# cdglissov/recurrent-flows-msc

Measured on AMD Instinct MI355X. Metric: frames/sec, RFN SM-MNIST 64x64 train step (fwd+bwd+Adam), higher is better.
Workload: dtype f32 (forward convolutions fp32-grade: fused scaled-fp16 split f16x3s / three-piece bf16x6 split; gradient convolutions bf16x3 split MFMA; fp32 accumulate everywhere); 1 GPU; RFN SM-MNIST 64x64 canonical (K=10 L=5 Hd=256 h=200 z=56), global_batch=32, seq_len=20, train step; global_batch=32, seq_len=20, parallelism=dp1

## Files before the change

### include/rfn_hip.h

```cpp
#ifndef RFN_HIP_H
#define RFN_HIP_H

#ifdef __cplusplus
extern "C" {
#endif

typedef void* rfn_stream_t;

int rfn_abi_version(void);
const char* rfn_last_error(void);

int rfn_squeeze2d_f32(const float* x, long x_ns, float* y, long y_ns, int N, int C, int H, int W, int undo,
                      rfn_stream_t stream);

int rfn_channel_stats_f32(const float* x, long x_ns, float* mean, float* var_unbiased, int N, int C, int HW,
                          rfn_stream_t stream);

int rfn_actnorm_invconv_fwd_f32(const float* x, long x_ns, const float* bias, const float* logs, const float* Wm,
                                float* z, long z_ns, int N, int C, int HW, rfn_stream_t stream);
int rfn_actnorm_invconv_bwd_f32(const float* x, long x_ns, const float* bias, const float* logs, const float* Wm,
                                const float* gz, long gz_ns, float* gx, long gx_ns, float* gW, float* gbias,
                                float* glogs, int N, int C, int HW, rfn_stream_t stream);
#define RFN_INVCONV_MAX_STEPS 32
#define RFN_INVCONV_MAX_CHANNELS 96
// ... 180 lines not shown
    const float* w;
    float* packed;
    int Cout, Cin, H, W, transpose, pad_;
} rfn_smallmap_pack_desc;
int rfn_smallmap_pack_batched_bf16x3(const void* descs_host, int n, rfn_stream_t stream);
int rfn_smallmap_dense_bf16x3(const float* a, const float* y, float slope_in, const float* packed, const float* bias,
                              const float* add, int act_out, float slope_out, float* out, float* a_out, int B, int K, int N,
                              int HW, rfn_stream_t stream);

int rfn_smallmap_dense_pair_bf16x3(const float* a0, const float* y0, float slope_in0, const float* packed0,
                                   const float* bias0, const float* add0, int act_out0, float slope_out0, float* out0,
                                   float* a_out0, int K0, int N0, const float* a1, const float* y1, float slope_in1,
                                   const float* packed1, const float* bias1, const float* add1, int act_out1,
                                   float slope_out1, float* out1, float* a_out1, int K1, int N1, int B, int HW,
                                   rfn_stream_t stream);

int rfn_smallmap_conv_bf16x3(const float* in1, long in1_ns, int C1, const float* in2, long in2_ns, int C2,
                             const float* packed, float* out1, long out1_ns, float* out2, long out2_ns, int Cout,
                             int cout_split, int acc1, int N, int H, int W, int ep_mode, const float* p0,
                             const float* p1, int act, rfn_stream_t stream);

long rfn_stepbn_scratch_floats(int S, int B, int C);
int rfn_stepbn_fwd_f32(const float* x, const float* gamma, const float* beta, float* y, float* mean, float* var, float* acc,
                       float* run_mean, float* run_var, const float* coef, const float* coef_u, float decay,
                       long long* num_batches_tracked, int S, int B, int C, int HW, float eps, int act, float slope,
                       rfn_stream_t stream);
int rfn_stepbn_bwd_f32(const float* x, const float* gamma, const float* beta, const float* g, const float* mean,
                       const float* var, float* sums, float* gx, float* ggamma, float* gbeta, int S, int B, int C, int HW,
                       float eps, int act, float slope, int stage, int world, rfn_stream_t stream);
int rfn_stepbn_apply_f32(const float* x, const float* gamma, const float* beta, float* y, const float* mean,
                         const float* var, int S, int B, int C, int HW, float eps, int act, float slope,
                         rfn_stream_t stream);
const char* rfn_stepbn_kernel_label(int S, int B, int C, int HW, int aligned, int bwd);

long rfn_bnflow_scratch_floats(int S, int B, int E, int bwd);
int rfn_bnflow_fwd_f32(const float* x, const float* log_gamma, const float* beta, float* z, float* mean, float* var,
                       float* dl, float* scratch, float* run_mean, float* run_var, const float* coef_mean,
                       const float* coef_var, float decay, int S, int B, int E, float eps, rfn_stream_t stream);
int rfn_bnflow_bwd_f32(const float* x, const float* log_gamma, const float* gz, const float* gdl, const float* mean,
                       const float* var, float* gx, float* g_log_gamma, float* g_beta, float* scratch, int S, int B,
                       int E, rfn_stream_t stream);
int rfn_bnflow_apply_f32(const float* x, const float* log_gamma, const float* beta, const float* run_mean,
                         const float* run_var, float* y, float* dl, int N, int E, int reverse, rfn_stream_t stream);

long rfn_mol_part_floats(int N, int HW);
int rfn_mol_nll_fwd(const float* x, const float* l, float* nll_pix, float* lse, float* nll, float* part, int N, int C, int M,
                    int HW, rfn_stream_t stream);
int rfn_mol_nll_bwd(const float* x, const float* l, const float* lse, const float* up, int up_per_pixel, float* dl, int N,
                    int C, int M, int HW, rfn_stream_t stream);
int rfn_mol_sample(const float* l, const float* u_mix, const float* u_x, float* out, int N, int C, int M, int HW,
                   rfn_stream_t stream);
int rfn_mol_sample_keyed(const float* l, float* out, int rows, int B, int C, int M, int HW, long seed, int step,
                         long first_seq, long first_draw, rfn_stream_t stream);
int rfn_mol_keyed_uniforms(float* u_mix, float* u_x, int rows, int B, int C, int M, int HW, long seed, int step,
                           long first_seq, long first_draw, rfn_stream_t stream);

const char* rfn_latent_step_kernel_label(int B, int ZHW);
const char* rfn_convlstm_gates_kernel_label(int N, int Hc, int HW);
int rfn_convlstm_gates_fwd_f32(const float* cc, const float* c_prev, long c_ns, const float* Wci, const float* Wcf,
                               const float* Wco, float* h_out, long h_ns, float* c_out, long co_ns, float* gates,
                               int N, int Hc, int HW, rfn_stream_t stream);
int rfn_convlstm_gates_bwd_f32(const float* gates, const float* c_prev, long c_ns, const float* c_out, long co_ns,
                               const float* gh, long gh_ns, const float* gc_next, long gcn_ns, const float* Wci,
                               const float* Wcf, const float* Wco, float* gcc, float* gc_prev, long gcp_ns, int N,
                               int Hc, int HW, rfn_stream_t stream);

// ... 72 lines not shown
```

### recurrent-flows-msc_amd/Utils/modules.py

```python
import os
from types import SimpleNamespace

import torch
import torch.nn as nn
import torch.nn.functional as F

from rfn_hip import ops as K


class ActFun(nn.Module):

    def __init__(self, non_lin, in_place=False):
        super().__init__()
        if non_lin == "relu":
            self.net = nn.ReLU(inplace=in_place)
        elif non_lin == "leakyrelu":
            self.net = nn.LeakyReLU(negative_slope=0.20, inplace=in_place)
        else:
            assert False, "Please specify a activation type from the set {relu,leakyrelu}"
        self.non_lin = non_lin

    def forward(self, x):
        return self.net(x)

# ... 38 lines not shown
            m = bn.momentum if bn.momentum is not None else 0.1
            coef = m * (1.0 - m) ** torch.arange(steps - 1, -1, -1, device=x.device, dtype=x.dtype)
            decay = (1.0 - m) ** steps
            bn.running_mean.mul_(decay).add_((coef.view(steps, 1) * tmp_m.view(steps, C)).sum(0))
            bn.running_var.mul_(decay).add_((coef.view(steps, 1) * tmp_v.view(steps, C)).sum(0))
            bn.num_batches_tracked += steps
    return y


def _act_code(m):
    if isinstance(m, ActFun):
        m = m.net
    if isinstance(m, nn.LeakyReLU):
        return 2, float(m.negative_slope)
    if isinstance(m, nn.ReLU):
        return 1, 0.0
    if isinstance(m, nn.Tanh):
        return 3, 0.0
    return None


_EMA_COEF = {}


def _ema_coef(steps, m, n, device):
    key = (steps, float(m), int(n), str(device))
    if key not in _EMA_COEF:
        c = m * (1.0 - m) ** torch.arange(steps - 1, -1, -1, dtype=torch.float64)
        _EMA_COEF[key] = (c.to(device=device, dtype=torch.float32),
                          (c * (n / max(n - 1, 1))).to(device=device, dtype=torch.float32))
    return _EMA_COEF[key]


def per_step_batchnorm_act(bn, x, steps, act_code, slope):
    running = None
    if bn.track_running_stats:
        n = (x.shape[0] // steps) * x.shape[2] * x.shape[3]
        m = bn.momentum if bn.momentum is not None else 0.1
        coef, coef_u = _ema_coef(steps, m, n, x.device)
        running = (bn.running_mean, bn.running_var, coef, coef_u, (1.0 - m) ** steps, bn.num_batches_tracked)
    y, _, _ = K.StepBatchNormActFn.apply(x, bn.weight if bn.affine else None, bn.bias if bn.affine else None, steps,
                                         float(bn.eps), act_code, slope, running)
    return y


def queue_conv_packs(seqs, x):
    packs = {}
    if x.is_cuda and x.dtype == torch.float32 and K.CONV_PRECISION != "f32" and K.bwd_b3():
        with K.PackBatch() as pb:
            for seq in seqs:
                for m in seq:
                    if _own_conv(m, x) and not K.fewcin_ok(x, None, m.weight, 0):
                        packs[m] = (pb.conv(m.weight, prec="bf16x6"),
                                    pb.conv(m.weight, flip=True) if torch.is_grad_enabled() else None)
    return packs


def run_time_batched(seq, x, steps, packs=None):
    mods = list(seq)
    if packs is None:
        packs = queue_conv_packs([seq], x)
    i = 0
    while i < len(mods):
        m = mods[i]
        if isinstance(m, NormLayer) and isinstance(m.norm, nn.BatchNorm2d):
            bn = m.norm
            fused = x.is_cuda and bn.training and x.dtype == torch.float32 and os.environ.get("RFN_STEPBN") != "0"
            if fused:
                act = _act_code(mods[i + 1]) if i + 1 < len(mods) else None
                x = per_step_batchnorm_act(bn, x, steps, act[0] if act else 0, act[1] if act else 0.0)
                i += 2 if act else 1
                continue
            x = per_step_batchnorm(bn, x, steps)
        elif _own_conv(m, x):
            x = K.conv_ep(x.contiguous(), None, m.weight, None, None, 0, 0,
                          prec="f32" if K.CONV_PRECISION == "f32" else "bf16x6", packs=packs.get(m))
        else:
            x = m(x)
        i += 1
    return x


def _own_conv(m, x):
    return (isinstance(m, nn.Conv2d) and x.is_cuda and x.dtype == torch.float32
            and tuple(m.kernel_size) == (3, 3) and tuple(m.stride) == (1, 1) and tuple(m.padding) == (1, 1)
            and tuple(m.dilation) == (1, 1) and m.groups == 1 and m.bias is None
            and os.environ.get("RFN_VGG_CONV", "own") != "miopen")


class Squeeze2dDecoder(nn.Module):

    def __init__(self, undo_squeeze=False):
        super().__init__()
        self.undo_squeeze = undo_squeeze

    def forward(self, x):
        return K.Squeeze2dFn.apply(x.contiguous(), self.undo_squeeze)


class _NearestUp2xFn(torch.autograd.Function):

    @staticmethod
    def forward(ctx, x):
        return torch.nn.functional.interpolate(x, scale_factor=2, mode="nearest")

    @staticmethod
    def backward(ctx, g):
        return torch.nn.functional.avg_pool2d(g, 2) * 4.0


class NearestUp2x(nn.Upsample):

    def __init__(self):
        super().__init__(scale_factor=2, mode="nearest")

    def forward(self, x):
        return _NearestUp2xFn.apply(x)


class tanh0_5(nn.Module):
    def forward(self, x):
        return 0.5 * torch.tanh(x)


def _conv_block(cin, cout, norm_type, act, stride=1):
    return [nn.Conv2d(cin, cout, kernel_size=3, stride=stride, padding=1, bias=False),
            NormLayer(cout, norm_type=norm_type), act]


class VGG_downscaler(nn.Module):

    def __init__(self, structures, L, in_channels, norm_type="batchnorm", non_lin="relu", scale=2, skip_con=False,
                 tanh=False):
        super().__init__()
        assert len(structures) == L, "Please specify number of blocks = L"
        self.l_nets = nn.ModuleList([])
        self.L, self.skip_con, self.scale = L, skip_con, scale
        for l, structure in enumerate(structures):
            layers = []
            for count, item in enumerate(structure, 1):
                last = count == len(structure)
                if l == L - 1 and last:
                    act = nn.Tanh()
                elif last and tanh:
                    act = tanh0_5()
                else:
                    act = ActFun(non_lin, in_place=True)
                if item == "pool":
                    layers.append(nn.MaxPool2d(kernel_size=2, stride=2))
                elif item == "conv":
# ... 71 lines not shown
                    in_channels = dc
                elif item == "squeeze":
                    dc = in_channels // 4
                    layer_up = [Squeeze2dDecoder(undo_squeeze=True), NormLayer(dc, norm_type=norm_type), act]
                    in_channels = dc
                else:
                    layers += [nn.Conv2d(in_channels + skip_channels, item, kernel_size=3, stride=1, padding=1,
                                         bias=False), NormLayer(item, norm_type=norm_type), act]
                    in_channels = item
            if l > 0:
                self.upscales_nets.append(nn.Sequential(*layer_up))
            self.net = nn.Sequential(*layers)
            self.l_nets.append(self.net)

    def forward(self, x, skip_list=None):
        outputs = []
        rev = list(reversed(skip_list)) if self.skips else None
        for i in range(self.L):
            if i > 0:
                x = self.upscales_nets[i - 1](x)
            if self.skips:
                x = self.l_nets[i](torch.cat((x, rev[i]), dim=1))
            else:
                x = self.l_nets[i](x)
            outputs.append(x)
        outputs.reverse()
        return outputs

    def forward_steps(self, x, steps, skip_list=None):
        outputs = []
        rev = list(reversed(skip_list)) if self.skips else None
        packs = queue_conv_packs(list(self.upscales_nets) + list(self.l_nets), x)
        for i in range(self.L):
            if i > 0:
                x = run_time_batched(self.upscales_nets[i - 1], x, steps, packs)
            if self.skips:
                x = torch.cat((x, rev[i]), dim=1)
            x = run_time_batched(self.l_nets[i], x, steps, packs)
            outputs.append(x)
        outputs.reverse()
        return outputs


class _StepStash:

    def __init__(self):
        self.xs, self.gs = [], []


class _WeightPort(torch.autograd.Function):

    @staticmethod
    def forward(ctx, w, b, stash):
        ctx.set_materialize_grads(False)
        ctx.stash, ctx.has_bias = stash, b is not None
        ctx.save_for_backward(w)
        return w.view_as(w), (b.view_as(b) if b is not None else None)

    @staticmethod
    def backward(ctx, _gw, _gb):
        (w,) = ctx.saved_tensors
        st = ctx.stash
        if not st.gs:
            return None, None, None
        X = st.xs[0] if len(st.xs) == 1 else torch.cat(st.xs, 0)
        G = st.gs[0] if len(st.gs) == 1 else torch.cat(st.gs, 0)
        st.xs, st.gs = [], []
        _, gw, gb = torch.ops.aten.convolution_backward(G, X, w, [w.shape[0]] if ctx.has_bias else None, [1, 1], [1, 1],
                                                        [1, 1], False, [0, 0], 1, [False, True, ctx.has_bias])
        return gw, (gb if ctx.has_bias else None), None
# ... 328 lines not shown
```

### recurrent-flows-msc_amd/csrc/shell.hip

```cpp
#include "common.h"
#include "../../include/rfn_hip.h"
#include <stdarg.h>

static thread_local char g_err[512] = "";
void rfn_set_error(const char* fmt, ...) {
    va_list ap;
    va_start(ap, fmt);
    vsnprintf(g_err, sizeof(g_err), fmt, ap);
    va_end(ap);
}
extern "C" const char* rfn_last_error(void) { return g_err; }
extern "C" int rfn_abi_version(void) { return 2; }

#include <map>
#include <mutex>
#include <vector>
float* rfn_workspace(hipStream_t s, size_t floats) {
    static std::mutex mu;
    static std::map<int, std::pair<float*, size_t>> tab;
    std::lock_guard<std::mutex> lock(mu);
    int dev = 0;
    (void)hipGetDevice(&dev);
    auto& e = tab[dev];
    if (e.second >= floats) return e.first;
// ... 1580 lines not shown
    if (threadIdx.x == 0) {
        float* dst = acc + ((long)blockIdx.y * gridDim.x + blockIdx.x) * 2;
        dst[0] = ta;
        dst[1] = tv;
    }
}
struct StepBnFused {
    const float* acc;
    float* mean_out;
    float* var_out;
    float* run_mean;
    float* run_var;
    const float* coef;
    const float* coef_u;
    float decay;
    long long* nbt;
    int S, ny;
};
__device__ __forceinline__ void stepbn_moments(const float* __restrict__ x, const float* __restrict__ acc, int sc, int s,
                                               int c, int B, int C, int HW, int ny, int SC, float& m, float& v) {
    if (!acc) return;
    const float K = x[((long)s * B * C + c) * HW];
    const float n = (float)B * HW;
    float s1 = 0.f, s2 = 0.f;
    for (int y = 0; y < ny; ++y) {
        s1 += acc[((long)y * SC + sc) * 2];
        s2 += acc[((long)y * SC + sc) * 2 + 1];
    }
    const float m1 = s1 / n;
    m = K + m1;
    const float vv = s2 / n - m1 * m1;
    v = vv > 0.f ? vv : 0.f;
}
template <int VEC>
__global__ void stepbn_apply_kernel(const float* __restrict__ x, const float* __restrict__ gamma,
                                    const float* __restrict__ beta, float* __restrict__ y, unsigned total, int B, int C,
                                    int HW, float eps, int act, float slope, StepBnFused f) {
    const int SC = f.S * C;
    const unsigned nblk = gridDim.x - 1, bid = blockIdx.x - 1;
    if (blockIdx.x == 0) {
        if (!f.acc) return;
        for (int sc = threadIdx.x; sc < SC; sc += blockDim.x) {
            float m, v;
            stepbn_moments(x, f.acc, sc, sc / C, sc % C, B, C, HW, f.ny, SC, m, v);
            f.mean_out[sc] = m;
            f.var_out[sc] = v;
        }
        if (f.run_mean) {
            for (int c = threadIdx.x; c < C; c += blockDim.x) {
                float em = 0.f, ev = 0.f;
#pragma unroll 4
                for (int s = 0; s < f.S; ++s) {
                    float m, v;
                    stepbn_moments(x, f.acc, s * C + c, s, c, B, C, HW, f.ny, SC, m, v);
                    em = fmaf(f.coef[s], m, em);
                    ev = fmaf(f.coef_u[s], v, ev);
                }
                f.run_mean[c] = fmaf(f.decay, f.run_mean[c], em);
                f.run_var[c] = fmaf(f.decay, f.run_var[c], ev);
            }
        }
        if (f.nbt && threadIdx.x == 0) *f.nbt += f.S;
        return;
    }
    const unsigned nvec = total / VEC;
    for (unsigned iv = bid * blockDim.x + threadIdx.x; iv < nvec; iv += nblk * blockDim.x) {
        const unsigned idx = iv * VEC;
        const unsigned r = idx / (unsigned)HW;
        const int c = (int)(r % (unsigned)C);
        const int s = (int)(r / (unsigned)C / (unsigned)B);
        float m = f.acc ? 0.f : f.mean_out[s * C + c], vr = f.acc ? 0.f : f.var_out[s * C + c];
        stepbn_moments(x, f.acc, s * C + c, s, c, B, C, HW, f.ny, SC, m, vr);
        const float rstd = rsqrtf(vr + eps);
        const float ga = gamma ? gamma[c] : 1.f, be = gamma ? beta[c] : 0.f;
        float v[VEC];
        if (VEC == 4) {
            const float4 t = *reinterpret_cast<const float4*>(x + idx);
            v[0] = t.x; v[1 % VEC] = t.y; v[2 % VEC] = t.z; v[3 % VEC] = t.w;
        } else {
            v[0] = x[idx];
        }
#pragma unroll
        for (int j = 0; j < VEC; ++j) v[j] = stepbn_act((v[j] - m) * rstd * ga + be, act, slope);
        if (VEC == 4)
            *reinterpret_cast<float4*>(y + idx) = float4{v[0], v[1 % VEC], v[2 % VEC], v[3 % VEC]};
        else
            y[idx] = v[0];
    }
}
__global__ __launch_bounds__(256) void stepbn_bwd_reduce_kernel(const float* __restrict__ x,
                                                                const float* __restrict__ gamma,
                                                                const float* __restrict__ beta,
                                                                const float* __restrict__ g,
                                                                const float* __restrict__ mean,
                                                                const float* __restrict__ var, float* __restrict__ sg,
// ... 8 lines not shown
    if ((HW & 3) == 0 && ((((uintptr_t)x) | ((uintptr_t)g)) & 15) == 0) {
        const int HW4 = HW >> 2, nb = (B - (int)blockIdx.y + (int)gridDim.y - 1) / (int)gridDim.y;
        for (int idx = threadIdx.x; idx < nb * HW4; idx += 256) {
            const int bi = idx / HW4, p = idx - bi * HW4;
            const long e0 = off + (blockIdx.y + (long)bi * gridDim.y) * fs;
            const float4 xq = reinterpret_cast<const float4*>(x + e0)[p], gq = reinterpret_cast<const float4*>(g + e0)[p];
            const float xv[4] = {xq.x, xq.y, xq.z, xq.w}, gv[4] = {gq.x, gq.y, gq.z, gq.w};
#pragma unroll
            for (int i = 0; i < 4; ++i) {
                const float xh = (xv[i] - m) * rstd;
                const float gp = gv[i] * stepbn_dact(xh * ga + be, act, slope);
                a += gp;
                ax = fmaf(gp, xh, ax);
            }
        }
    } else {
        for (int b = blockIdx.y; b < B; b += gridDim.y) {
            const long e0 = off + b * fs;
            for (int p = threadIdx.x; p < HW; p += 256) {
                const float xh = (x[e0 + p] - m) * rstd;
                const float gp = g[e0 + p] * stepbn_dact(xh * ga + be, act, slope);
                a += gp;
                ax = fmaf(gp, xh, ax);
            }
        }
    }
    const float ta = block_sum_256(a, sm);
    const float tx = block_sum_256(ax, sm);
    if (threadIdx.x == 0) {
        sg[(long)blockIdx.y * gridDim.x + blockIdx.x] = ta;
        sgx[(long)blockIdx.y * gridDim.x + blockIdx.x] = tx;
    }
}
template <int VEC>
__global__ void stepbn_bwd_apply_kernel(const float* __restrict__ x, const float* __restrict__ beta,
                                        const float* __restrict__ g, const float* __restrict__ mean,
                                        const float* __restrict__ var, const float* __restrict__ gamma,
                                        const float* __restrict__ sg, const float* __restrict__ sgx,
                                        float* __restrict__ gx, unsigned total, int B, int C, int HW, float eps, int act,
                                        float slope, float* __restrict__ ggamma, float* __restrict__ gbeta, int S, int ny,
                                        int world) {
    const int SC = S * C;
    const unsigned nblk = ggamma ? gridDim.x - 1 : gridDim.x, bid = ggamma ? blockIdx.x - 1 : blockIdx.x;
    if (ggamma && blockIdx.x == 0) {
        for (int c = threadIdx.x; c < C; c += blockDim.x) {
            float a = 0.f, b = 0.f;
            for (int i = 0; i < ny * S; ++i) {
                a += sgx[(long)i * C + c];
                b += sg[(long)i * C + c];
            }
            ggamma[c] = a / (float)world;
            gbeta[c] = b / (float)world;
        }
        return;
    }
    const float inv_n = 1.f / ((float)(B * HW) * (float)world);
    const unsigned nvec = total / VEC;
    for (unsigned iv = bid * blockDim.x + threadIdx.x; iv < nvec; iv += nblk * blockDim.x) {
        const unsigned idx = iv * VEC;
        const unsigned r = idx / (unsigned)HW;
        const int c = (int)(r % (unsigned)C);
        const int s = (int)(r / (unsigned)C / (unsigned)B);
        const int sc = s * C + c;
        const float rstd = rsqrtf(var[sc] + eps), m = mean[sc];
        const float w = gamma ? gamma[c] : 1.f, be = gamma ? beta[c] : 0.f;
        float k1 = 0.f, k2 = 0.f;
        for (int yy = 0; yy < ny; ++yy) {
            k1 += sg[(long)yy * SC + sc];
            k2 += sgx[(long)yy * SC + sc];
        }
        k1 *= inv_n;
        k2 *= inv_n;
        float xv[VEC], gv[VEC];
        if (VEC == 4) {
            const float4 t = *reinterpret_cast<const float4*>(x + idx);
            const float4 u = *reinterpret_cast<const float4*>(g + idx);
            xv[0] = t.x; xv[1 % VEC] = t.y; xv[2 % VEC] = t.z; xv[3 % VEC] = t.w;
            gv[0] = u.x; gv[1 % VEC] = u.y; gv[2 % VEC] = u.z; gv[3 % VEC] = u.w;
        } else {
            xv[0] = x[idx];
            gv[0] = g[idx];
        }
#pragma unroll
        for (int j = 0; j < VEC; ++j) {
            const float xh = (xv[j] - m) * rstd;
            const float gp = gv[j] * stepbn_dact(xh * w + be, act, slope);
// ... 84 lines not shown
        hipLaunchKernelGGL(stepbn_apply_kernel<1>, dim3(grid + 1), dim3(256), 0, (hipStream_t)stream, x, gamma, beta, y,
                           (unsigned)total, B, C, HW, eps, act, slope, f);
    RFN_LAUNCH_CHECK();
    return 0;
}
extern "C" int rfn_stepbn_bwd_f32(const float* x, const float* gamma, const float* beta, const float* g, const float* mean,
                                  const float* var, float* sums, float* gx, float* ggamma, float* gbeta, int S, int B,
                                  int C, int HW, float eps, int act, float slope, int stage, int world,
                                  rfn_stream_t stream) {
    RFN_CHECK_ARG(x && g && mean && var && sums && gx && S > 0 && B > 0 && C > 0 && HW > 0, -1);
    RFN_CHECK_ARG(stage >= 0 && stage <= 2 && world >= 1, -4);
    RFN_CHECK_ARG(((gamma && beta) || (!gamma && !beta)) && ((ggamma && gbeta) || (!ggamma && !gbeta)), -2);
    const long total = (long)S * B * C * HW;
    RFN_CHECK_ARG(total < (1L << 31), -3);
    hipStream_t st = (hipStream_t)stream;
    const StepBnRoute r = choose_stepbn(S, B, C, HW, stepbn_aligned(x, g, x, g, gx));
    const int ny = r.ny, grid = r.grid;
    float* sg = sums;
    float* sgx = sums + (long)ny * S * C;
    if (stage != 2)
        hipLaunchKernelGGL(stepbn_bwd_reduce_kernel, dim3(S * C, ny), dim3(256), 0, st, x, gamma, beta, g, mean, var, sg, sgx,
                           B, C, HW, eps, act, slope);
    if (stage == 1) {
        RFN_LAUNCH_CHECK();
        return 0;
    }
    const int extra = ggamma ? 1 : 0;
    if (r.v4)
        hipLaunchKernelGGL(stepbn_bwd_apply_kernel<4>, dim3(grid + extra), dim3(256), 0, st, x, beta, g, mean, var, gamma,
                           sg, sgx, gx, (unsigned)total, B, C, HW, eps, act, slope, ggamma, gbeta, S, ny, world);
    else
        hipLaunchKernelGGL(stepbn_bwd_apply_kernel<1>, dim3(grid + extra), dim3(256), 0, st, x, beta, g, mean, var, gamma,
                           sg, sgx, gx, (unsigned)total, B, C, HW, eps, act, slope, ggamma, gbeta, S, ny, world);
    RFN_LAUNCH_CHECK();
    return 0;
}

struct InvConvWeightsParams {
    const float* p[RFN_INVCONV_MAX_STEPS];
    const float* lower[RFN_INVCONV_MAX_STEPS];
    const float* upper[RFN_INVCONV_MAX_STEPS];
    const float* log_s[RFN_INVCONV_MAX_STEPS];
    const float* sign_s[RFN_INVCONV_MAX_STEPS];
    float* W;
    float* logdet;
    const float* gW;
    const float* gc;
    float* g_lower;
    float* g_upper;
    float* g_log_s;
    int C;
    float hw;
};
__device__ __forceinline__ void invconv_load_LU(const InvConvWeightsParams& q, int k, float* Lm, float* Um) {
    const int C = q.C, CP = C + 1;
    for (int i = threadIdx.x; i < C * C; i += blockDim.x) {
        const int r = i / C, c = i - r * C;
        Lm[r * CP + c] = r > c ? q.lower[k][i] : (r == c ? 1.f : 0.f);
        Um[r * CP + c] = r < c ? q.upper[k][i] : (r == c ? q.sign_s[k][r] * expf(q.log_s[k][r]) : 0.f);
    }
}
__device__ __forceinline__ void invconv_load(const float* __restrict__ src, float* dst, int C) {
    for (int i = threadIdx.x; i < C * C; i += blockDim.x) dst[(i / C) * (C + 1) + i % C] = src[i];
}
template <bool TA, bool TB, typename Store>
__device__ __forceinline__ void invconv_mm(const float* __restrict__ A, const float* __restrict__ B, int C, Store store) {
// ... 318 lines not shown
```

### recurrent-flows-msc_amd/rfn_hip/ops.py

```python
import collections
import ctypes
import functools
import itertools

import torch

from . import lib as L

import os

CONV_PRECISION = os.environ.get("RFN_CONV_PRECISION", "mixed")


def bwd_b3():
    return CONV_PRECISION in ("bf16x3", "mixed")


MIXED_FWD = os.environ.get("RFN_MIXED_FWD", "bf16x6")


def fwd_prec(H, W):
    if CONV_PRECISION == "mixed":
        return "bf16x3" if H * W <= 4 else MIXED_FWD
    return CONV_PRECISION
# ... 1480 lines not shown
            n = B * HW * world
            cfu_g = cf * (n / max(n - 1, 1))
            rm.mul_(decay).add_((cf.view(-1, 1) * mean).sum(0))
            rv.mul_(decay).add_((cfu_g.view(-1, 1) * var).sum(0))
            if nbt is not None:
                nbt.add_(S)
        ctx.save_for_backward(x, mean, var, gm, bt)
        ctx.cfg = (S, B, C, HW, eps, act, slope, gamma is not None, nscr)
        ctx.world = world
        ctx.mark_non_differentiable(mean, var)
        return y, mean, var

    @staticmethod
    def backward(ctx, g, _gm, _gv):
        x, mean, var, gm, bt = ctx.saved_tensors
        S, B, C, HW, eps, act, slope, affine, nscr = ctx.cfg
        if g is None:
            return (None,) * 8
        g = g.contiguous()
        sums = torch.empty((nscr,), device=x.device, dtype=torch.float32)
        gx = torch.empty_like(x)
        ggamma = torch.empty((C,), device=x.device, dtype=torch.float32) if affine else None
        gbeta = torch.empty((C,), device=x.device, dtype=torch.float32) if affine else None
        args = (L.dev(x), L.dev(gm), L.dev(bt), L.dev(g), L.dev(mean), L.dev(var), L.dev(sums), L.dev(gx), L.dev(ggamma),
                L.dev(gbeta), S, B, C, HW, eps, act, slope)
        if ctx.world > 1:
            from . import dist as rdist
            L.call("rfn_stepbn_bwd_f32", *args, 1, ctx.world)
            rdist.all_reduce_sum_(sums)
            L.call("rfn_stepbn_bwd_f32", *args, 2, ctx.world)
        else:
            L.call("rfn_stepbn_bwd_f32", *args, 0, 1)
        return gx, ggamma, gbeta, None, None, None, None, None


def bnflow_coef(steps, momentum):
    m = float(momentum)
    coef = (1.0 - m) * torch.tensor([m ** (steps - 1 - s) for s in range(steps)], dtype=torch.float64)
    return coef, m ** steps


class BatchNormFlowFn(torch.autograd.Function):

    @staticmethod
    def forward(ctx, x, log_gamma, beta, steps, eps, running=None):
        x = x.contiguous()
        S, B = int(steps), int(x.shape[0]) // int(steps)
        E = x[0].numel()
        if S * B != x.shape[0] or log_gamma.numel() != E or beta.numel() != E:
            raise RuntimeError("BatchNormFlowFn: x %s is not %d steps of rows of %d elements" % (tuple(x.shape), S, log_gamma.numel()))
        lg, bt = _f(log_gamma), _f(beta)
        z = torch.empty_like(x)
        mean = torch.empty((S, E), device=x.device, dtype=torch.float32)
        var = torch.empty((S, E), device=x.device, dtype=torch.float32)
        dl = torch.empty((S,), device=x.device, dtype=torch.float32)
        scr = torch.empty((int(L.load().rfn_bnflow_scratch_floats(S, B, E, 0)),), device=x.device, dtype=torch.float32)
        rm = rv = cf = None
        decay = 1.0
        if running is not None:
            rm, rv, cf, decay = running
            if not (rm.is_contiguous() and rv.is_contiguous()) or rm.numel() != E or rv.numel() != E or cf.numel() != S:
                raise RuntimeError("BatchNormFlowFn: running statistics must be dense [%d] tensors, coef [%d]" % (E, S))
        L.call("rfn_bnflow_fwd_f32", L.dev(x), L.dev(lg), L.dev(bt), L.dev(z), L.dev(mean), L.dev(var), L.dev(dl),
               L.dev(scr), L.dev(rm), L.dev(rv), L.dev(cf), L.dev(cf), decay, S, B, E,
               eps, meta=_shell("bnflow_fwd", x, 2))
        ctx.save_for_backward(x, lg, mean, var)
# ... 460 lines not shown
```

Before: 11790 frames/s.

## Fuse per-step BatchNorm+activation with 2x2 maxpool and upsample with skip concat

Adds fused kernels that apply per-step batchnorm, the activation and a 2x2 max-pool in one pass, recomputing the pooling argmax in backward instead of materialising the full-resolution activation. A second fused kernel performs nearest 2x upsampling and channel concatenation with the skip tensor in a single write, with a matching backward that sums the 2x2 gradient blocks. The goal is to cut intermediate full-size tensors and extra kernel launches in the encoder and decoder paths. In exchange, backward recomputes the normalisation and winner selection, and both paths are gated on layer patterns and environment variables.

```diff
diff --git a/include/rfn_hip.h b/include/rfn_hip.h
--- a/include/rfn_hip.h
+++ b/include/rfn_hip.h
@@ -236,6 +236,19 @@
                          const float* var, int S, int B, int C, int HW, float eps, int act, float slope,
                          rfn_stream_t stream);
 const char* rfn_stepbn_kernel_label(int S, int B, int C, int HW, int aligned, int bwd);
+int rfn_stepbn_pool_fwd_f32(const float* x, const float* gamma, const float* beta, float* p, float* mean, float* var,
+                            float* acc, float* run_mean, float* run_var, const float* coef, const float* coef_u,
+                            float decay, long long* num_batches_tracked, int S, int B, int C, int H, int W, float eps,
+                            int act, float slope, rfn_stream_t stream);
+int rfn_stepbn_pool_bwd_f32(const float* x, const float* gamma, const float* beta, const float* gp, const float* mean,
+                            const float* var, float* sums, float* gx, float* ggamma, float* gbeta, int S, int B, int C,
+                            int H, int W, float eps, int act, float slope, int stage, int world, rfn_stream_t stream);
+const char* rfn_stepbn_pool_kernel_label(int S, int B, int C, int H, int W, int aligned, int bwd);
+
+int rfn_up2x_cat_f32(const float* x, long x_ns, const float* skip, long skip_ns, float* out, int N, int Cx, int Cs, int h,
+                     int w, rfn_stream_t stream);
+int rfn_up2x_cat_bwd_f32(const float* g, long g_ns, float* gx, int N, int Cx, int h, int w, rfn_stream_t stream);
+const char* rfn_up2x_cat_kernel_label(int N, int Cx, int Cs, int h, int w, int aligned, int bwd);
 
 long rfn_bnflow_scratch_floats(int S, int B, int E, int bwd);
 int rfn_bnflow_fwd_f32(const float* x, const float* log_gamma, const float* beta, float* z, float* mean, float* var,
diff --git a/recurrent-flows-msc_amd/Utils/modules.py b/recurrent-flows-msc_amd/Utils/modules.py
--- a/recurrent-flows-msc_amd/Utils/modules.py
+++ b/recurrent-flows-msc_amd/Utils/modules.py
@@ -94,15 +94,31 @@
     return _EMA_COEF[key]
 
 
-def per_step_batchnorm_act(bn, x, steps, act_code, slope):
+def _pool2x2(m):
+    pair = lambda v: tuple(v) if isinstance(v, (tuple, list)) else (v, v)
+    return (type(m) is nn.MaxPool2d and pair(m.kernel_size) == (2, 2) and pair(m.stride) == (2, 2)
+            and pair(m.padding) == (0, 0) and pair(m.dilation) == (1, 1) and not m.ceil_mode and not m.return_indices)
+
+
+def _pool_fusable(mods, i, x):
+    if os.environ.get("RFN_STEPBN_POOL") == "0" or i + 2 >= len(mods) or _act_code(mods[i + 1]) is None:
+        return False
+    if not _pool2x2(mods[i + 2]) or x.shape[2] % 2 or x.shape[3] % 2:
+        return False
+    from rfn_hip import dist as rdist
+    return not rdist.sync_batchnorm_on()
+
+
+def per_step_batchnorm_act(bn, x, steps, act_code, slope, pool=False):
     running = None
     if bn.track_running_stats:
         n = (x.shape[0] // steps) * x.shape[2] * x.shape[3]
         m = bn.momentum if bn.momentum is not None else 0.1
         coef, coef_u = _ema_coef(steps, m, n, x.device)
         running = (bn.running_mean, bn.running_var, coef, coef_u, (1.0 - m) ** steps, bn.num_batches_tracked)
-    y, _, _ = K.StepBatchNormActFn.apply(x, bn.weight if bn.affine else None, bn.bias if bn.affine else None, steps,
-                                         float(bn.eps), act_code, slope, running)
+    fn = K.StepBatchNormActPoolFn if pool else K.StepBatchNormActFn
+    y, _, _ = fn.apply(x, bn.weight if bn.affine else None, bn.bias if bn.affine else None, steps, float(bn.eps),
+                       act_code, slope, running)
     return y
 
 
@@ -130,8 +146,9 @@
             fused = x.is_cuda and bn.training and x.dtype == torch.float32 and os.environ.get("RFN_STEPBN") != "0"
             if fused:
                 act = _act_code(mods[i + 1]) if i + 1 < len(mods) else None
-                x = per_step_batchnorm_act(bn, x, steps, act[0] if act else 0, act[1] if act else 0.0)
-                i += 2 if act else 1
+                pool = _pool_fusable(mods, i, x)
+                x = per_step_batchnorm_act(bn, x, steps, act[0] if act else 0, act[1] if act else 0.0, pool)
+                i += 3 if pool else 2 if act else 1
                 continue
             x = per_step_batchnorm(bn, x, steps)
         elif _own_conv(m, x):
@@ -178,6 +195,13 @@
 
     def forward(self, x):
         return _NearestUp2xFn.apply(x)
+
+
+def _up2x_only(seq, x, skip):
+    return (len(seq) == 1 and type(seq[0]) is NearestUp2x and x.is_cuda and skip.is_cuda and x.dtype == torch.float32
+            and skip.dtype == torch.float32 and x.dim() == 4 and skip.dim() == 4 and skip.shape[1] > 0
+            and tuple(skip.shape[2:]) == (2 * x.shape[2], 2 * x.shape[3]) and skip.shape[0] == x.shape[0]
+            and os.environ.get("RFN_UP2X_CAT") != "0")
 
 
 class tanh0_5(nn.Module):
@@ -315,10 +339,13 @@
         rev = list(reversed(skip_list)) if self.skips else None
         packs = queue_conv_packs(list(self.upscales_nets) + list(self.l_nets), x)
         for i in range(self.L):
-            if i > 0:
-                x = run_time_batched(self.upscales_nets[i - 1], x, steps, packs)
-            if self.skips:
-                x = torch.cat((x, rev[i]), dim=1)
+            if i > 0 and self.skips and _up2x_only(self.upscales_nets[i - 1], x, rev[i]):
+                x = K.Up2xCatFn.apply(x, rev[i])
+            else:
+                if i > 0:
+                    x = run_time_batched(self.upscales_nets[i - 1], x, steps, packs)
+                if self.skips:
+                    x = torch.cat((x, rev[i]), dim=1)
             x = run_time_batched(self.l_nets[i], x, steps, packs)
             outputs.append(x)
         outputs.reverse()
diff --git a/recurrent-flows-msc_amd/csrc/shell.hip b/recurrent-flows-msc_amd/csrc/shell.hip
--- a/recurrent-flows-msc_amd/csrc/shell.hip
+++ b/recurrent-flows-msc_amd/csrc/shell.hip
@@ -1636,6 +1636,31 @@
     const float vv = s2 / n - m1 * m1;
     v = vv > 0.f ? vv : 0.f;
 }
+__device__ __forceinline__ void stepbn_finalise(const float* __restrict__ x, int B, int C, int HW, const StepBnFused& f) {
+    const int SC = f.S * C;
+    if (!f.acc) return;
+    for (int sc = threadIdx.x; sc < SC; sc += blockDim.x) {
+        float m, v;
+        stepbn_moments(x, f.acc, sc, sc / C, sc % C, B, C, HW, f.ny, SC, m, v);
+        f.mean_out[sc] = m;
+        f.var_out[sc] = v;
+    }
+    if (f.run_mean) {
+        for (int c = threadIdx.x; c < C; c += blockDim.x) {
+            float em = 0.f, ev = 0.f;
+#pragma unroll 4
+            for (int s = 0; s < f.S; ++s) {
+                float m, v;
+                stepbn_moments(x, f.acc, s * C + c, s, c, B, C, HW, f.ny, SC, m, v);
+                em = fmaf(f.coef[s], m, em);
+                ev = fmaf(f.coef_u[s], v, ev);
+            }
+            f.run_mean[c] = fmaf(f.decay, f.run_mean[c], em);
+            f.run_var[c] = fmaf(f.decay, f.run_var[c], ev);
+        }
+    }
+    if (f.nbt && threadIdx.x == 0) *f.nbt += f.S;
+}
 template <int VEC>
 __global__ void stepbn_apply_kernel(const float* __restrict__ x, const float* __restrict__ gamma,
                                     const float* __restrict__ beta, float* __restrict__ y, unsigned total, int B, int C,
@@ -1643,28 +1668,7 @@
     const int SC = f.S * C;
     const unsigned nblk = gridDim.x - 1, bid = blockIdx.x - 1;
     if (blockIdx.x == 0) {
-        if (!f.acc) return;
-        for (int sc = threadIdx.x; sc < SC; sc += blockDim.x) {
-            float m, v;
-            stepbn_moments(x, f.acc, sc, sc / C, sc % C, B, C, HW, f.ny, SC, m, v);
-            f.mean_out[sc] = m;
-            f.var_out[sc] = v;
-        }
-        if (f.run_mean) {
-            for (int c = threadIdx.x; c < C; c += blockDim.x) {
-                float em = 0.f, ev = 0.f;
-#pragma unroll 4
-                for (int s = 0; s < f.S; ++s) {
-                    float m, v;
-                    stepbn_moments(x, f.acc, s * C + c, s, c, B, C, HW, f.ny, SC, m, v);
-                    em = fmaf(f.coef[s], m, em);
-                    ev = fmaf(f.coef_u[s], v, ev);
-                }
-                f.run_mean[c] = fmaf(f.decay, f.run_mean[c], em);
-                f.run_var[c] = fmaf(f.decay, f.run_var[c], ev);
-            }
-        }
-        if (f.nbt && threadIdx.x == 0) *f.nbt += f.S;
+        stepbn_finalise(x, B, C, HW, f);
         return;
     }
     const unsigned nvec = total / VEC;
@@ -1739,6 +1743,19 @@
         sgx[(long)blockIdx.y * gridDim.x + blockIdx.x] = tx;
     }
 }
+__device__ __forceinline__ void stepbn_param_grads(const float* __restrict__ sg, const float* __restrict__ sgx,
+                                                   float* __restrict__ ggamma, float* __restrict__ gbeta, int C, int S,
+                                                   int ny, int world) {
+    for (int c = threadIdx.x; c < C; c += blockDim.x) {
+        float a = 0.f, b = 0.f;
+        for (int i = 0; i < ny * S; ++i) {
+            a += sgx[(long)i * C + c];
+            b += sg[(long)i * C + c];
+        }
+        ggamma[c] = a / (float)world;
+        gbeta[c] = b / (float)world;
+    }
+}
 template <int VEC>
 __global__ void stepbn_bwd_apply_kernel(const float* __restrict__ x, const float* __restrict__ beta,
                                         const float* __restrict__ g, const float* __restrict__ mean,
@@ -1750,15 +1767,7 @@
     const int SC = S * C;
     const unsigned nblk = ggamma ? gridDim.x - 1 : gridDim.x, bid = ggamma ? blockIdx.x - 1 : blockIdx.x;
     if (ggamma && blockIdx.x == 0) {
-        for (int c = threadIdx.x; c < C; c += blockDim.x) {
-            float a = 0.f, b = 0.f;
-            for (int i = 0; i < ny * S; ++i) {
-                a += sgx[(long)i * C + c];
-                b += sg[(long)i * C + c];
-            }
-            ggamma[c] = a / (float)world;
-            gbeta[c] = b / (float)world;
-        }
+        stepbn_param_grads(sg, sgx, ggamma, gbeta, C, S, ny, world);
         return;
     }
     const float inv_n = 1.f / ((float)(B * HW) * (float)world);
@@ -1909,6 +1918,375 @@
     else
         hipLaunchKernelGGL(stepbn_bwd_apply_kernel<1>, dim3(grid + extra), dim3(256), 0, st, x, beta, g, mean, var, gamma,
                            sg, sgx, gx, (unsigned)total, B, C, HW, eps, act, slope, ggamma, gbeta, S, ny, world);
+    RFN_LAUNCH_CHECK();
+    return 0;
+}
+
+__device__ __forceinline__ int stepbn_pool_winner(const float xv[4], float m, float rstd, float ga, float be, int act,
+                                                  float slope, float& best, float& xh_w, float& u_w) {
+    int k = 0;
+#pragma unroll
+    for (int j = 0; j < 4; ++j) {
+        const float xh = (xv[j] - m) * rstd;
+        const float u = xh * ga + be;
+        const float a = stepbn_act(u, act, slope);
+        if (j == 0 || a > best || isnan(a)) {
+            best = a;
+            xh_w = xh;
+            u_w = u;
+            k = j;
+        }
+    }
+    return k;
+}
+template <int VEC>
+__device__ __forceinline__ void stepbn_pool_load(const float* __restrict__ x, unsigned in0, int W, float xv[2][4]) {
+    if (VEC == 4) {
+        const float4 r0 = *reinterpret_cast<const float4*>(x + in0);
+        const float4 r1 = *reinterpret_cast<const float4*>(x + in0 + W);
+        xv[0][0] = r0.x; xv[0][1] = r0.y; xv[0][2] = r1.x; xv[0][3] = r1.y;
+        xv[1][0] = r0.z; xv[1][1] = r0.w; xv[1][2] = r1.z; xv[1][3] = r1.w;
+    } else {
+        xv[0][0] = x[in0]; xv[0][1] = x[in0 + 1]; xv[0][2] = x[in0 + W]; xv[0][3] = x[in0 + W + 1];
+    }
+}
+template <int VEC>
+__global__ void stepbn_pool_apply_kernel(const float* __restrict__ x, const float* __restrict__ gamma,
+                                         const float* __restrict__ beta, float* __restrict__ p, unsigned nunits, int B,
+                                         int C, int H, int W, float eps, int act, float slope, StepBnFused f) {
+    constexpr int NW = VEC == 4 ? 2 : 1;
+    const int SC = f.S * C, HW = H * W;
+    const unsigned nblk = gridDim.x - 1, bid = blockIdx.x - 1;
+    if (blockIdx.x == 0) {
+        stepbn_finalise(x, B, C, HW, f);
+        return;
+    }
+    const unsigned upr = (unsigned)W / (2 * NW), Ho = (unsigned)H / 2;
+    for (unsigned u = bid * blockDim.x + threadIdx.x; u < nunits; u += nblk * blockDim.x) {
+        const unsigned q = u / upr;
+        const unsigned r = q / Ho;
+        const int c = (int)(r % (unsigned)C);
+        const int s = (int)(r / (unsigned)C / (unsigned)B);
+        float m = f.acc ? 0.f : f.mean_out[s * C + c], vr = f.acc ? 0.f : f.var_out[s * C + c];
+        stepbn_moments(x, f.acc, s * C + c, s, c, B, C, HW, f.ny, SC, m, vr);
+        const float rstd = rsqrtf(vr + eps);
+        const float ga = gamma ? gamma[c] : 1.f, be = gamma ? beta[c] : 0.f;
+        float xv[2][4], o[NW];
+        stepbn_pool_load<VEC>(x, q * 2u * (unsigned)W + 2u * NW * (u - q * upr), W, xv);
+#pragma unroll
+        for (int w = 0; w < NW; ++w) {
+            float xh, uu;
+            stepbn_pool_winner(xv[w], m, rstd, ga, be, act, slope, o[w], xh, uu);
+        }
+        if (VEC == 4)
+            *reinterpret_cast<float2*>(p + 2u * u) = float2{o[0], o[NW - 1]};
+        else
+            p[u] = o[0];
+    }
+}
+__device__ __forceinline__ double block_sum_256_f64(double v, double* sm ) {
+#pragma unroll
+    for (int o = 32; o > 0; o >>= 1) v += __shfl_xor(v, o, 64);
+    const int lane = threadIdx.x & 63, wave = threadIdx.x >> 6;
+    __syncthreads();
+    if (lane == 0) sm[wave] = v;
+    __syncthreads();
+    return (sm[0] + sm[1]) + (sm[2] + sm[3]);
+}
+template <int VEC>
+__global__ __launch_bounds__(256) void stepbn_pool_bwd_reduce_kernel(
+    const float* __restrict__ x, const float* __restrict__ gamma, const float* __restrict__ beta,
+    const float* __restrict__ gp, const float* __restrict__ mean, const float* __restrict__ var, float* __restrict__ sg,
+    float* __restrict__ sgx, int B, int C, int H, int W, float eps, int act, float slope) {
+    constexpr int NW = VEC == 4 ? 2 : 1;
+    __shared__ double sm[4];
+    const int s = blockIdx.x / C, c = blockIdx.x - s * C;
+    const int HW = H * W, upr = W / (2 * NW), upf = (H / 2) * upr;
+    const unsigned pl0 = (unsigned)(s * B) * C + c;
+    const float m = mean[blockIdx.x], rstd = rsqrtf(var[blockIdx.x] + eps);
+    const float ga = gamma ? gamma[c] : 1.f, be = gamma ? beta[c] : 0.f;
+    double a = 0., ax = 0.;
+    const int nb = (B - (int)blockIdx.y + (int)gridDim.y - 1) / (int)gridDim.y;
+    for (int idx = threadIdx.x; idx < nb * upf; idx += 256) {
+        const int bi = idx / upf, t = idx - bi * upf;
+        const unsigned pl = pl0 + (blockIdx.y + (unsigned)bi * gridDim.y) * (unsigned)C;
+        const int i = t / upr, j = t - i * upr;
+        float xv[2][4], gv[NW];
+        stepbn_pool_load<VEC>(x, pl * (unsigned)HW + 2u * i * W + 2u * NW * j, W, xv);
+        const unsigned o0 = pl * (unsigned)(HW / 4) + (unsigned)t * NW;
+        if (VEC == 4) {
+            const float2 g2 = *reinterpret_cast<const float2*>(gp + o0);
+            gv[0] = g2.x; gv[NW - 1] = g2.y;
+        } else {
+            gv[0] = gp[o0];
+        }
+#pragma unroll
+        for (int w = 0; w < NW; ++w) {
+            float best, xh, u;
+            stepbn_pool_winner(xv[w], m, rstd, ga, be, act, slope, best, xh, u);
+            const float g1 = gv[w] * stepbn_dact(u, act, slope);
+            a += (double)g1;
+            ax = fma((double)g1, (double)xh, ax);
+        }
+    }
+    const float ta = (float)block_sum_256_f64(a, sm);
+    const float tx = (float)block_sum_256_f64(ax, sm);
+    if (threadIdx.x == 0) {
+        sg[(long)blockIdx.y * gridDim.x + blockIdx.x] = ta;
+        sgx[(long)blockIdx.y * gridDim.x + blockIdx.x] = tx;
+    }
+}
+template <int VEC>
+__global__ void stepbn_pool_bwd_apply_kernel(const float* __restrict__ x, const float* __restrict__ beta,
+                                             const float* __restrict__ gp, const float* __restrict__ mean,
+                                             const float* __restrict__ var, const float* __restrict__ gamma,
+                                             const float* __restrict__ sg, const float* __restrict__ sgx,
+                                             float* __restrict__ gx, unsigned nunits, int B, int C, int H, int W,
+                                             float eps, int act, float slope, float* __restrict__ ggamma,
+                                             float* __restrict__ gbeta, int S, int ny, int world) {
+    constexpr int NW = VEC == 4 ? 2 : 1;
+    const int SC = S * C, HW = H * W;
+    const unsigned nblk = ggamma ? gridDim.x - 1 : gridDim.x, bid = ggamma ? blockIdx.x - 1 : blockIdx.x;
+    if (ggamma && blockIdx.x == 0) {
+        stepbn_param_grads(sg, sgx, ggamma, gbeta, C, S, ny, world);
+        return;
+    }
+    const float inv_n = 1.f / ((float)(B * HW) * (float)world);
+    const unsigned upr = (unsigned)W / (2 * NW), Ho = (unsigned)H / 2;
+    for (unsigned u = bid * blockDim.x + threadIdx.x; u < nunits; u += nblk * blockDim.x) {
+        const unsigned q = u / upr;
+        const unsigned r = q / Ho;
+        const int c = (int)(r % (unsigned)C);
+        const int s = (int)(r / (unsigned)C / (unsigned)B);
+        const int sc = s * C + c;
+        const float rstd = rsqrtf(var[sc] + eps), m = mean[sc];
+        const float w = gamma ? gamma[c] : 1.f, be = gamma ? beta[c] : 0.f;
+        float k1 = 0.f, k2 = 0.f;
+        for (int yy = 0; yy < ny; ++yy) {
+            k1 += sg[(long)yy * SC + sc];
+            k2 += sgx[(long)yy * SC + sc];
+        }
+        k1 *= inv_n;
+        k2 *= inv_n;
+        const unsigned in0 = q * 2u * (unsigned)W + 2u * NW * (u - q * upr);
+        float xv[2][4], gv[NW];
+        stepbn_pool_load<VEC>(x, in0, W, xv);
+        if (VEC == 4) {
+            const float2 g2 = *reinterpret_cast<const float2*>(gp + 2u * u);
+            gv[0] = g2.x; gv[NW - 1] = g2.y;
+        } else {
+            gv[0] = gp[u];
+        }
+#pragma unroll
+        for (int ww = 0; ww < NW; ++ww) {
+            float best, xhw, uw;
+            const int k = stepbn_pool_winner(xv[ww], m, rstd, w, be, act, slope, best, xhw, uw);
+            const float g1 = gv[ww] * stepbn_dact(uw, act, slope);
+#pragma unroll
+            for (int j = 0; j < 4; ++j) {
+                const float xh = (xv[ww][j] - m) * rstd;
+                const float gpos = j == k ? g1 : 0.f;
+                xv[ww][j] = w * rstd * (gpos - k1 - xh * k2);
+            }
+        }
+        if (VEC == 4) {
+            *reinterpret_cast<float4*>(gx + in0) = float4{xv[0][0], xv[0][1], xv[NW - 1][0], xv[NW - 1][1]};
+            *reinterpret_cast<float4*>(gx + in0 + W) = float4{xv[0][2], xv[0][3], xv[NW - 1][2], xv[NW - 1][3]};
+        } else {
+            gx[in0] = xv[0][0]; gx[in0 + 1] = xv[0][1]; gx[in0 + W] = xv[0][2]; gx[in0 + W + 1] = xv[0][3];
+        }
+    }
+}
+constexpr int STEPBN_POOL_GRID_CAP = 8192;
+struct StepBnPoolRoute {
+    int ny;
+    bool stats_vec;
+    bool v4;
+    long nunits;
+    int grid;
+    int sweeps;
+};
+static StepBnPoolRoute choose_stepbn_pool(int S, int B, int C, int H, int W, int aligned, int bwd) {
+    StepBnPoolRoute r;
+    const long total = (long)S * B * C * H * W;
+    r.ny = stepbn_split(S, B, C);
+    r.stats_vec = (aligned & 1) && (bwd ? W % 4 == 0 : true);
+    r.v4 = W % 4 == 0 && (aligned & 2);
+    r.nunits = r.v4 ? total / 8 : total / 4;
+    const long nb = (r.nunits + 255) / 256;
+    r.grid = (int)(nb < STEPBN_POOL_GRID_CAP ? nb : STEPBN_POOL_GRID_CAP);
+    r.sweeps = (int)((nb + r.grid - 1) / r.grid);
+    return r;
+}
+static bool stepbn_pool_sizes_ok(int S, int B, int C, int H, int W) {
+    return S > 0 && B > 0 && C > 0 && H > 0 && W > 0 && H % 2 == 0 && W % 2 == 0;
+}
+extern "C" const char* rfn_stepbn_pool_kernel_label(int S, int B, int C, int H, int W, int aligned, int bwd) {
+    static thread_local char buf[160];
+    if (!stepbn_pool_sizes_ok(S, B, C, H, W) || (long)S * B * C * H * W >= (1L << 31)) return "unsupported";
+    const StepBnPoolRoute r = choose_stepbn_pool(S, B, C, H, W, aligned, bwd);
+    snprintf(buf, sizeof(buf), "stepbn_pool ny=%d stats=%s apply=%s grid=%d sweeps=%d", r.ny,
+             r.stats_vec ? "vec" : "scalar", r.v4 ? "vec4" : "vec1", r.grid, r.sweeps);
+    return buf;
+}
+extern "C" int rfn_stepbn_pool_fwd_f32(const float* x, const float* gamma, const float* beta, float* p, float* mean,
+                                       float* var, float* acc, float* run_mean, float* run_var, const float* coef,
+                                       const float* coef_u, float decay, long long* nbt, int S, int B, int C, int H, int W,
+                                       float eps, int act, float slope, rfn_stream_t stream) {
+    RFN_CHECK_ARG(x && p && mean && var && acc && S > 0 && B > 0 && C > 0 && H > 0 && W > 0, -1);
+    RFN_CHECK_ARG(((gamma && beta) || (!gamma && !beta)) && ((run_mean && run_var && coef && coef_u) || (!run_mean && !run_var)),
+                  -2);
+    RFN_CHECK_ARG(H % 2 == 0 && W % 2 == 0, -5);
+    const long total = (long)S * B * C * H * W;
+    RFN_CHECK_ARG(total < (1L << 31), -3);
+    hipStream_t st = (hipStream_t)stream;
+    const StepBnPoolRoute r = choose_stepbn_pool(S, B, C, H, W, stepbn_aligned(x, nullptr, x, p, nullptr), 0);
+    hipLaunchKernelGGL(stepbn_stats_kernel, dim3(S * C, r.ny), dim3(256), 0, st, x, acc, B, C, H * W);
+    StepBnFused f;
+    f.acc = acc; f.mean_out = mean; f.var_out = var; f.run_mean = run_mean; f.run_var = run_var; f.coef = coef;
+    f.coef_u = coef_u; f.decay = decay; f.nbt = nbt; f.S = S; f.ny = r.ny;
+    if (r.v4)
+        hipLaunchKernelGGL(stepbn_pool_apply_kernel<4>, dim3(r.grid + 1), dim3(256), 0, st, x, gamma, beta, p,
+                           (unsigned)r.nunits, B, C, H, W, eps, act, slope, f);
+    else
+        hipLaunchKernelGGL(stepbn_pool_apply_kernel<1>, dim3(r.grid + 1), dim3(256), 0, st, x, gamma, beta, p,
+                           (unsigned)r.nunits, B, C, H, W, eps, act, slope, f);
+    RFN_LAUNCH_CHECK();
+    return 0;
+}
+extern "C" int rfn_stepbn_pool_bwd_f32(const float* x, const float* gamma, const float* beta, const float* gp,
+                                       const float* mean, const float* var, float* sums, float* gx, float* ggamma,
+                                       float* gbeta, int S, int B, int C, int H, int W, float eps, int act, float slope,
+                                       int stage, int world, rfn_stream_t stream) {
+    RFN_CHECK_ARG(x && gp && mean && var && sums && gx && S > 0 && B > 0 && C > 0 && H > 0 && W > 0, -1);
+    RFN_CHECK_ARG(stage >= 0 && stage <= 2 && world >= 1, -4);
+    RFN_CHECK_ARG(((gamma && beta) || (!gamma && !beta)) && ((ggamma && gbeta) || (!ggamma && !gbeta)), -2);
+    RFN_CHECK_ARG(H % 2 == 0 && W % 2 == 0, -5);
+    const long total = (long)S * B * C * H * W;
+    RFN_CHECK_ARG(total < (1L << 31), -3);
+    hipStream_t st = (hipStream_t)stream;
+    const StepBnPoolRoute r = choose_stepbn_pool(S, B, C, H, W, stepbn_aligned(x, gp, x, gp, gx), 1);
+    const int ny = r.ny;
+    float* sg = sums;
+    float* sgx = sums + (long)ny * S * C;
+    if (stage != 2) {
+        if (r.stats_vec)
+            hipLaunchKernelGGL(stepbn_pool_bwd_reduce_kernel<4>, dim3(S * C, ny), dim3(256), 0, st, x, gamma, beta, gp, mean,
+                               var, sg, sgx, B, C, H, W, eps, act, slope);
+        else
+            hipLaunchKernelGGL(stepbn_pool_bwd_reduce_kernel<1>, dim3(S * C, ny), dim3(256), 0, st, x, gamma, beta, gp, mean,
+                               var, sg, sgx, B, C, H, W, eps, act, slope);
+    }
+    if (stage == 1) {
+        RFN_LAUNCH_CHECK();
+        return 0;
+    }
+    const int extra = ggamma ? 1 : 0;
+    if (r.v4)
+        hipLaunchKernelGGL(stepbn_pool_bwd_apply_kernel<4>, dim3(r.grid + extra), dim3(256), 0, st, x, beta, gp, mean, var,
+                           gamma, sg, sgx, gx, (unsigned)r.nunits, B, C, H, W, eps, act, slope, ggamma, gbeta, S, ny, world);
+    else
+        hipLaunchKernelGGL(stepbn_pool_bwd_apply_kernel<1>, dim3(r.grid + extra), dim3(256), 0, st, x, beta, gp, mean, var,
+                           gamma, sg, sgx, gx, (unsigned)r.nunits, B, C, H, W, eps, act, slope, ggamma, gbeta, S, ny, world);
+    RFN_LAUNCH_CHECK();
+    return 0;
+}
+
+constexpr int UP2X_GRID_CAP = 8192;
+template <int VEC>
+__global__ void up2x_cat_kernel(const float* __restrict__ x, long x_ns, const float* __restrict__ skip, long s_ns,
+                                float* __restrict__ out, unsigned nunits, int Cx, int Cs, int h, int w) {
+    const unsigned upr = VEC == 4 ? (unsigned)w / 2 : 2u * w, H2 = 2u * h, Ct = (unsigned)(Cx + Cs);
+    for (unsigned u = blockIdx.x * blockDim.x + threadIdx.x; u < nunits; u += gridDim.x * blockDim.x) {
+        const unsigned row = u / upr, k = u - row * upr;
+        const unsigned rc = row / H2, Y = row - rc * H2;
+        const unsigned n = rc / Ct, c = rc - n * Ct;
+        if (VEC == 4) {
+            float4 v;
+            if (c < (unsigned)Cx) {
+                const float2 t = *reinterpret_cast<const float2*>(x + n * x_ns + ((long)c * h + Y / 2) * w + 2 * k);
+                v = float4{t.x, t.x, t.y, t.y};
+            } else {
+                v = *reinterpret_cast<const float4*>(skip + n * s_ns + ((long)(c - Cx) * H2 + Y) * (2 * w) + 4 * k);
+            }
+            *reinterpret_cast<float4*>(out + 4ul * u) = v;
+        } else {
+            out[u] = c < (unsigned)Cx ? x[n * x_ns + ((long)c * h + Y / 2) * w + k / 2]
+                                      : skip[n * s_ns + ((long)(c - Cx) * H2 + Y) * (2 * w) + k];
+        }
+    }
+}
+template <int VEC>
+__global__ void up2x_cat_bwd_kernel(const float* __restrict__ g, long g_ns, float* __restrict__ gx, unsigned nunits,
+                                    int Cx, int h, int w) {
+    const unsigned upr = VEC == 4 ? (unsigned)w / 2 : (unsigned)w;
+    for (unsigned u = blockIdx.x * blockDim.x + threadIdx.x; u < nunits; u += gridDim.x * blockDim.x) {
+        const unsigned row = u / upr, k = u - row * upr;
+        const unsigned rc = row / (unsigned)h, i = row - rc * (unsigned)h;
+        const unsigned n = rc / (unsigned)Cx, c = rc - n * (unsigned)Cx;
+        const float* r0 = g + n * g_ns + ((long)c * 2 * h + 2 * i) * (2 * w) + (VEC == 4 ? 4 : 2) * k;
+        const float* r1 = r0 + 2 * w;
+        if (VEC == 4) {
+            const float4 a = *reinterpret_cast<const float4*>(r0), b = *reinterpret_cast<const float4*>(r1);
+            *reinterpret_cast<float2*>(gx + 2ul * u) = float2{(float)(((double)a.x + a.y) + ((double)b.x + b.y)),
+                                                              (float)(((double)a.z + a.w) + ((double)b.z + b.w))};
+        } else {
+            gx[u] = (float)(((double)r0[0] + r0[1]) + ((double)r1[0] + r1[1]));
+        }
+    }
+}
+struct Up2xRoute {
+    bool v4;
+    long nunits;
+    int grid, sweeps;
+};
+static Up2xRoute choose_up2x(long out_elems, int w, int aligned, int bwd) {
+    Up2xRoute r;
+    r.v4 = w % 2 == 0 && aligned;
+    r.nunits = r.v4 ? out_elems / (bwd ? 2 : 4) : out_elems;
+    const long nb = (r.nunits + 255) / 256;
+    r.grid = (int)(nb < UP2X_GRID_CAP ? nb : UP2X_GRID_CAP);
+    r.sweeps = (int)((nb + r.grid - 1) / r.grid);
+    return r;
+}
+static bool up2x_sizes_ok(int N, int Cx, int Cs, int h, int w, int bwd) {
+    return N > 0 && Cx > 0 && Cs >= 0 && h > 0 && w > 0 && 4L * N * (bwd ? Cx : Cx + Cs) * h * w < (1L << 31);
+}
+extern "C" const char* rfn_up2x_cat_kernel_label(int N, int Cx, int Cs, int h, int w, int aligned, int bwd) {
+    static thread_local char buf[128];
+    if (!up2x_sizes_ok(N, Cx, Cs, h, w, bwd)) return "unsupported";
+    const Up2xRoute r = choose_up2x(bwd ? (long)N * Cx * h * w : 4L * N * (Cx + Cs) * h * w, w, aligned, bwd);
+    snprintf(buf, sizeof(buf), "up2x_cat%s access=%s grid=%d sweeps=%d", bwd ? "_bwd" : "", r.v4 ? "vec4" : "vec1", r.grid,
+             r.sweeps);
+    return buf;
+}
+extern "C" int rfn_up2x_cat_f32(const float* x, long x_ns, const float* skip, long skip_ns, float* out, int N, int Cx,
+                                int Cs, int h, int w, rfn_stream_t stream) {
+    RFN_CHECK_ARG(x && skip && out && Cs > 0 && up2x_sizes_ok(N, Cx, Cs, h, w, 0), -1);
+    RFN_CHECK_ARG(x_ns >= (long)Cx * h * w && skip_ns >= 4L * Cs * h * w, -2);
+    const int aligned = ((((uintptr_t)x | (uintptr_t)skip | (uintptr_t)out) & 15) == 0 && x_ns % 4 == 0 && skip_ns % 4 == 0);
+    const Up2xRoute r = choose_up2x(4L * N * (Cx + Cs) * h * w, w, aligned, 0);
+    if (r.v4)
+        hipLaunchKernelGGL(up2x_cat_kernel<4>, dim3(r.grid), dim3(256), 0, (hipStream_t)stream, x, x_ns, skip, skip_ns, out,
+                           (unsigned)r.nunits, Cx, Cs, h, w);
+    else
+        hipLaunchKernelGGL(up2x_cat_kernel<1>, dim3(r.grid), dim3(256), 0, (hipStream_t)stream, x, x_ns, skip, skip_ns, out,
+                           (unsigned)r.nunits, Cx, Cs, h, w);
+    RFN_LAUNCH_CHECK();
+    return 0;
+}
+extern "C" int rfn_up2x_cat_bwd_f32(const float* g, long g_ns, float* gx, int N, int Cx, int h, int w,
+                                    rfn_stream_t stream) {
+    RFN_CHECK_ARG(g && gx && up2x_sizes_ok(N, Cx, 0, h, w, 1), -1);
+    RFN_CHECK_ARG(g_ns >= 4L * Cx * h * w, -2);
+    const int aligned = ((((uintptr_t)g | (uintptr_t)gx) & 15) == 0 && g_ns % 4 == 0);
+    const Up2xRoute r = choose_up2x((long)N * Cx * h * w, w, aligned, 1);
+    if (r.v4)
+        hipLaunchKernelGGL(up2x_cat_bwd_kernel<4>, dim3(r.grid), dim3(256), 0, (hipStream_t)stream, g, g_ns, gx,
+                           (unsigned)r.nunits, Cx, h, w);
+    else
+        hipLaunchKernelGGL(up2x_cat_bwd_kernel<1>, dim3(r.grid), dim3(256), 0, (hipStream_t)stream, g, g_ns, gx,
+                           (unsigned)r.nunits, Cx, h, w);
     RFN_LAUNCH_CHECK();
     return 0;
 }
diff --git a/recurrent-flows-msc_amd/rfn_hip/ops.py b/recurrent-flows-msc_amd/rfn_hip/ops.py
--- a/recurrent-flows-msc_amd/rfn_hip/ops.py
+++ b/recurrent-flows-msc_amd/rfn_hip/ops.py
@@ -1536,6 +1536,83 @@
         else:
             L.call("rfn_stepbn_bwd_f32", *args, 0, 1)
         return gx, ggamma, gbeta, None, None, None, None, None
+
+
+class StepBatchNormActPoolFn(torch.autograd.Function):
+
+    @staticmethod
+    def forward(ctx, x, gamma, beta, S, eps, act, slope, running=None):
+        ctx.set_materialize_grads(False)
+        x = x.contiguous()
+        SB, C, H, W = (int(v) for v in x.shape)
+        B = SB // S
+        mean = torch.empty((S, C), device=x.device, dtype=torch.float32)
+        var = torch.empty((S, C), device=x.device, dtype=torch.float32)
+        p = torch.empty((SB, C, H // 2, W // 2), device=x.device, dtype=torch.float32)
+        gm = None if gamma is None else gamma.detach().contiguous()
+        bt = None if beta is None else beta.detach().contiguous()
+        nscr = int(L.load().rfn_stepbn_scratch_floats(S, B, C))
+        acc = torch.empty((nscr,), device=x.device, dtype=torch.float32)
+        rm = rv = cf = cfu = nbt = None
+        decay = 1.0
+        if running is not None:
+            rm, rv, cf, cfu, decay, nbt = running
+            if nbt is not None and (nbt.dtype != torch.int64 or not nbt.is_cuda):
+                raise RuntimeError("num_batches_tracked must be an int64 device tensor")
+        L.call("rfn_stepbn_pool_fwd_f32", L.dev(x), L.dev(gm), L.dev(bt), L.dev(p), L.dev(mean), L.dev(var), L.dev(acc),
+               L.dev(rm), L.dev(rv), L.dev(cf), L.dev(cfu), decay, None if nbt is None else nbt.data_ptr(), S, B, C, H, W,
+               eps, act, slope, meta=_shell("stepbn_pool_fwd", x, 2.25))
+        ctx.save_for_backward(x, mean, var, gm, bt)
+        ctx.cfg = (S, B, C, H, W, eps, act, slope, gamma is not None, nscr)
+        ctx.mark_non_differentiable(mean, var)
+        return p, mean, var
+
+    @staticmethod
+    def backward(ctx, gp, _gm, _gv):
+        x, mean, var, gm, bt = ctx.saved_tensors
+        S, B, C, H, W, eps, act, slope, affine, nscr = ctx.cfg
+        if gp is None:
+            return (None,) * 8
+        gp = gp.contiguous()
+        sums = torch.empty((nscr,), device=x.device, dtype=torch.float32)
+        gx = torch.empty_like(x)
+        ggamma = torch.empty((C,), device=x.device, dtype=torch.float32) if affine else None
+        gbeta = torch.empty((C,), device=x.device, dtype=torch.float32) if affine else None
+        L.call("rfn_stepbn_pool_bwd_f32", L.dev(x), L.dev(gm), L.dev(bt), L.dev(gp), L.dev(mean), L.dev(var), L.dev(sums),
+               L.dev(gx), L.dev(ggamma), L.dev(gbeta), S, B, C, H, W, eps, act, slope, 0, 1,
+               meta=_shell("stepbn_pool_bwd", x, 3.5))
+        return gx, ggamma, gbeta, None, None, None, None, None
+
+
+class Up2xCatFn(torch.autograd.Function):
+
+    @staticmethod
+    def forward(ctx, x, skip):
+        N, Cx, h, w = (int(v) for v in x.shape)
+        Cs = int(skip.shape[1])
+        if tuple(skip.shape) != (N, Cs, 2 * h, 2 * w):
+            raise RuntimeError("Up2xCatFn: skip %s does not fit x %s" % (tuple(skip.shape), tuple(x.shape)))
+        dense = lambda t: all(t.shape[d] == 1 or t.stride(d) == e for d, e in
+                              ((3, 1), (2, t.shape[3]), (1, t.shape[2] * t.shape[3])))
+        x, skip = (t if dense(t) else t.contiguous() for t in (x, skip))
+        xp, xns = L.frames(x, "x")
+        sp, sns = L.frames(skip, "skip")
+        out = torch.empty((N, Cx + Cs, 2 * h, 2 * w), device=x.device, dtype=torch.float32)
+        L.call("rfn_up2x_cat_f32", xp, xns, sp, sns, L.dev(out), N, Cx, Cs, h, w,
+               meta=_shell("up2x_cat", out, 1.0 + (0.25 * Cx + Cs) / (Cx + Cs)))
+        ctx.cfg = (N, Cx, h, w)
+        return out
+
+    @staticmethod
+    def backward(ctx, g):
+        N, Cx, h, w = ctx.cfg
+        g = g.contiguous()
+        gx = None
+        if ctx.needs_input_grad[0]:
+            gp, gns = L.frames(g, "g")
+            gx = torch.empty((N, Cx, h, w), device=g.device, dtype=torch.float32)
+            L.call("rfn_up2x_cat_bwd_f32", gp, gns, L.dev(gx), N, Cx, h, w, meta=_shell("up2x_cat_bwd", gx, 5))
+        return gx, (g[:, Cx:] if ctx.needs_input_grad[1] else None)
 
 
 def bnflow_coef(steps, momentum):
```

After: 12000 frames/s (median of 6 runs). 1.02x the previous value.
